# darrenjkt/SEE-VCN

Hardware: AMD Instinct MI355X
Metric: scenes/sec (VCN+voxel+spconv fwd+bwd) (higher is better)
Workload: dtype f32; 1 GPU; VCN_VC fwd on 64 objects x 1024 pts -> kNN surface select (k=30) -> largest DBSCAN cluster (eps 0.4) -> unique + replace (<0.1 m) into 16 KITTI-shaped 64-beam scenes (21.0k pts in range each) -> DynMeanVFE -> VoxelBackBone8x + HeightCompression fwd+bwd + SGD (BASELINE configs[1]+[2]); scenes_per_gpu=16, objects_per_gpu=64, points_per_object=1024, geometry=KITTI [0,-40,-3,70.4,40,1] @ [0.05,0.05,0.1] -> sparse [41,1600,1408], parallelism=dp1, input_side=side stream, one batch ahead (every step = 1 front + 1 compute)

## Files before the change

include/seevcn_hip.h:

```cpp
#ifndef SEEVCN_HIP_H
#define SEEVCN_HIP_H

#include <stddef.h>
#include <stdint.h>

#ifdef __cplusplus
extern "C" {
#endif

#define SV_OK 0
#define SV_ERR_ARG 1
#define SV_ERR_HIP 2

#define SV_ABI_VERSION 1

int sv_abi_version(void);
const char* sv_last_error(void);
int sv_measure_build(void);

size_t sv_index_persistent_bytes(int64_t ncells);
size_t sv_index_scratch_bytes(int64_t ncells);

size_t sv_voxelize_dynamic_scratch_bytes(int64_t num_points, int64_t ncells, int64_t capacity);
int sv_voxelize_dynamic(const float* points, int64_t num_points, int point_stride, int num_features,
// ... 293 lines not shown
int sv_weighted_smooth_l1_loss(const float* input, const float* target, const float* code_weights, const float* weights, int64_t n_rows,
                               int num_codes, float beta, const float* grad_out, float* out, void* stream);

int sv_center_assign_targets(const float* gt_boxes, int batch, int max_gt, int box_dim, int num_heads, int num_class,
                             const int32_t* cls_to_local, const int32_t* head_num_class, const int32_t* head_cls_offset, int total_cls,
                             int fm_w, int fm_h, float x_min, float y_min, float voxel_x, float voxel_y, float fm_stride,
                             int num_max_objs, float gaussian_overlap, int min_radius, float* heatmaps, float* target_boxes,
                             int64_t* inds, int64_t* masks, void* stream);

int sv_ball_query_batch(int batch, int n, int m, float radius, int nsample, const float* new_xyz, const float* xyz, int32_t* idx,
                        void* stream);
int sv_group_points_batch(int batch, int c, int n, int npoints, int nsample, const float* points, const int32_t* idx, float* out,
                          void* stream);
int sv_group_points_grad_batch(int batch, int c, int n, int npoints, int nsample, const float* grad_out, const int32_t* idx,
                               float* grad_points, void* stream);
int sv_gather_points_batch(int batch, int c, int n, int npoints, const float* points, const int32_t* idx, float* out, void* stream);
int sv_gather_points_grad_batch(int batch, int c, int n, int npoints, const float* grad_out, const int32_t* idx, float* grad_points,
                                void* stream);
int sv_three_nn_batch(int batch, int n, int m, const float* unknown, const float* known, float* dist2, int32_t* idx, void* stream);
int sv_three_interpolate_batch(int batch, int c, int m, int n, const float* points, const int32_t* idx, const float* weight, float* out,
                               void* stream);
int sv_three_interpolate_grad_batch(int batch, int c, int n, int m, const float* grad_out, const int32_t* idx, const float* weight,
                                    float* grad_points, void* stream);
size_t sv_group_points_grad_batch_ordered_scratch_bytes(int batch, int n, int npoints, int nsample);
int sv_group_points_grad_batch_ordered(int batch, int c, int n, int npoints, int nsample, const float* grad_out, const int32_t* idx,
                                       void* scratch, float* grad_points, void* stream);
size_t sv_gather_points_grad_batch_ordered_scratch_bytes(int batch, int n, int npoints);
int sv_gather_points_grad_batch_ordered(int batch, int c, int n, int npoints, const float* grad_out, const int32_t* idx, void* scratch,
                                        float* grad_points, void* stream);
size_t sv_three_interpolate_grad_batch_ordered_scratch_bytes(int batch, int n, int m);
int sv_three_interpolate_grad_batch_ordered(int batch, int c, int n, int m, const float* grad_out, const int32_t* idx, const float* weight,
                                            void* scratch, float* grad_points, void* stream);

#define SV_OP_WORDS 32
#define SV_OP_CONV_PLANNED 1
#define SV_OP_CONV_PLAIN 2
#define SV_OP_BN_FWD 3
#define SV_OP_BN_BWD 5
#define SV_OP_WGRAD 6
#define SV_OP_DGRAD_PLANNED_BN 7
#define SV_OP_WGRAD_DEFERRED 8
#define SV_OP_BN_FINALIZE 9
#define SV_OP_BN_APPLY 10
#define SV_OP_BN_STATS_LOCAL 11
#define SV_OP_BN_FINALIZE_GLOBAL 12
#define SV_OP_BN_BWD_SUMS_LOCAL 13
#define SV_OP_BN_BWD_APPLY_GLOBAL 14
#define SV_OP_BN_EVAL_COEF_BATCH 15
#define SV_OP_CONV_PLANNED_H16 16
#define SV_OP_NARROW_H16 17
int sv_run_ops(const int64_t* ops, int n_ops, void* stream);
int sv_run_ops_timed(const int64_t* ops, int n_ops, void* stream, float* ms);
int sv_run_ops_two_streams(const int64_t* ops, int n_ops, void* stream, void* side_stream);

size_t sv_batchnorm_scratch_bytes(int channels);
int sv_batchnorm_relu_forward(const float* x, int64_t n, int channels, const float* gamma, const float* beta, float* running_mean,
                              float* running_var, float momentum, float eps, int training, int relu, void* scratch, float* y,
                              float* save_mean, float* save_invstd, int64_t* num_batches_tracked, void* stream);
int sv_batchnorm_relu_forward_partial(const float* x, int64_t n, int channels, const float* gamma, const float* beta, float* running_mean,
                                      float* running_var, float momentum, float eps, int relu, void* scratch, int n_partials, float* y,
                                      float* save_mean, float* save_invstd, int64_t* num_batches_tracked, void* stream);
int sv_batchnorm_finalize_forward(const float* x , int64_t n, int channels, const float* gamma, const float* beta, float* running_mean, float* running_var,
                                  float momentum, float eps, void* scratch, int n_partials, float* coef, float* save_mean, float* save_invstd,
                                  int64_t* num_batches_tracked, void* stream);
int sv_batchnorm_eval_coef_batch(const int64_t* jobs_host, int n_jobs, void* stream);
int sv_batchnorm_apply(const float* x, int64_t n, int channels, const float* coef, int relu, float* y, void* stream);
int sv_batchnorm_relu_backward(const float* x, const float* dy, int64_t n, int channels, const float* gamma, const float* beta,
                               const float* save_mean, const float* save_invstd, int relu, void* scratch, float* dx, float* dgamma,
                               float* dbeta, void* stream);
int sv_batchnorm_relu_backward_partial(const float* x, const float* dy, int64_t n, int channels, const float* gamma, const float* beta,
                                       const float* save_mean, const float* save_invstd, int relu, void* scratch, int n_partials, float* dx,
                                       float* dgamma, float* dbeta, void* stream);
int sv_batchnorm_stats_local(const float* x, int64_t n, int channels, void* scratch, int n_partials, double* sums, void* stream);
int sv_batchnorm_finalize_global(const double* gathered, int world, int channels, const float* gamma, const float* beta, float* running_mean,
                                 float* running_var, float momentum, float eps, float* coef, float* save_mean, float* save_invstd,
                                 int64_t* num_batches_tracked, double* total_rows, void* stream);
int sv_batchnorm_backward_sums_local(const float* x, const float* dy, int64_t n, int channels, const float* gamma, const float* beta,
                                     const float* save_mean, const float* save_invstd, int relu, void* scratch, int n_partials, float* dgamma,
                                     float* dbeta, double* sums, void* stream);
int sv_batchnorm_backward_apply_global(const float* x, const float* dy, int64_t n, int channels, const float* gamma, const float* beta,
                                       const float* save_mean, const float* save_invstd, int relu, const double* gathered, int world,
                                       const double* total_rows, void* scratch, float* dx, void* stream);

int sv_gemm_bias_act_ragged(const float* A, int lda, const float* W, int ldw, const float* bias, const float* group_bias,
                            const int32_t* row_group, float* C, int ldc, float* group_max, int M, int N, int K, int act, float slope,
                            void* stream);
int sv_gemm_bias_act_ragged_dev(const float* A, int lda, const float* W, int ldw, const float* bias, const float* group_bias,
                                const int32_t* row_group, float* C, int ldc, float* group_max, int M_cap, const int32_t* m_dev, int N, int K,
                                int act, float slope, void* stream);
int sv_unique_rows(const float* x, int batch, int n, int32_t* uniq_idx, int32_t* counts, void* stream);
int sv_unique_rows_compact(const int32_t* uniq_idx, const int32_t* counts, int batch, int n, int64_t* sel, int32_t* row_group,
                           int32_t* total, void* stream);

int sv_chamfer_forward(const float* xyz1, const float* xyz2, int batch, int n, int m, float* dist1, float* dist2, int32_t* idx1,
                       int32_t* idx2, void* stream);
int sv_chamfer_backward(const float* xyz1, const float* xyz2, const int32_t* idx1, const int32_t* idx2, const float* grad_dist1,
                        const float* grad_dist2, int batch, int n, int m, float* grad_xyz1, float* grad_xyz2, void* stream);
size_t sv_chamfer_backward_ordered_scratch_bytes(int batch, int n, int m);
int sv_chamfer_backward_ordered(const float* xyz1, const float* xyz2, const int32_t* idx1, const int32_t* idx2, const float* grad_dist1,
                                const float* grad_dist2, int batch, int n, int m, void* scratch, float* grad_xyz1, float* grad_xyz2,
                                void* stream);

size_t sv_vcn_surface_select_scratch_bytes(int batch);
int sv_vcn_surface_select(const float* partial, const float* complete, int batch, int n_partial, int n_complete, int k,
                          int surface_pts, void* scratch, float* surface, int32_t* n_selected, void* stream);
int sv_vcn_largest_cluster(const float* points, int batch, int n, double eps, int min_points, int total_pts, float* out,
// ... 162 lines not shown
```

see-vcn_amd/_lib.py:

```python
import ctypes
import os

import torch

_HERE = os.path.dirname(os.path.abspath(__file__))
LIB_PATH = os.environ.get("SEEVCN_LIB") or os.path.join(_HERE, "lib", "libseevcn_hip.so")
HEADER_PATH = os.path.join(os.path.dirname(_HERE), "include", "seevcn_hip.h")

c_p = ctypes.c_void_p
c_i = ctypes.c_int
c_i64 = ctypes.c_int64
c_f = ctypes.c_float
c_d = ctypes.c_double
c_sz = ctypes.c_size_t

SIGNATURES = {
    "sv_abi_version": (c_i, []),
    "sv_last_error": (ctypes.c_char_p, []),
    "sv_measure_build": (c_i, []),
    "sv_index_persistent_bytes": (c_sz, [c_i64]),
    "sv_index_scratch_bytes": (c_sz, [c_i64]),
    "sv_voxelize_dynamic_scratch_bytes": (c_sz, [c_i64, c_i64, c_i64]),
    "sv_voxelize_dynamic": (c_i, [c_p, c_i64, c_i, c_i, c_p, c_p, c_p, c_i, c_p, c_p, c_p, c_p, c_p, c_i64, c_p, c_p]),
    "sv_mean_vfe": (c_i, [c_p, c_p, c_i64, c_i, c_i, c_p, c_p]),
# ... 153 lines not shown
    "sv_dedup_rows_scratch_bytes": (c_sz, [c_i64]),
    "sv_dedup_rows": (c_i, [c_p, c_i64, c_p, c_p]),
    "sv_points_near_set": (c_i, [c_p, c_i64, c_p, c_i64, c_i, c_d, c_p, c_p]),
    "sv_points_near_set_scratch_bytes": (c_sz, [c_i64]),
    "sv_points_near_set_boxed": (c_i, [c_p, c_i64, c_p, c_i64, c_i, c_d, c_p, c_p, c_p]),
    "sv_points_in_boxes_matrix": (c_i, [c_p, c_p, c_i, c_i, c_p, c_p]),
    "sv_crop_points_in_boxes": (c_i, [c_p, c_i64, c_i, c_p, c_i, c_i64, c_p, c_p, c_p]),
    "sv_project_lidar_to_image_kitti": (c_i, [c_p, c_i64, c_i, c_p, c_p, c_p, c_i, c_i, c_d, c_p, c_p, c_p, c_p]),
    "sv_project_lidar_to_image_camera": (c_i, [c_p, c_i64, c_i, c_p, c_p, c_p, c_i, c_i, c_i, c_p, c_p, c_p, c_p]),
    "sv_project_lidar_to_image_nuscenes": (c_i, [c_p, c_i64, c_i, c_p, c_p, c_p, c_i, c_i, c_d, c_p, c_p, c_p, c_p]),
    "sv_polygon_masks_scratch_bytes": (c_sz, [c_i, c_i, c_i]),
    "sv_polygons_to_masks": (c_i, [c_p, c_p, c_p, c_i, c_i, c_i, c_i, c_i, c_p, c_p, c_p]),
    "sv_polygons_to_masks_shrunk": (c_i, [c_p, c_p, c_p, c_p, c_i, c_i, c_i, c_i, c_i, c_p, c_p, c_p, c_p]),
    "sv_points_in_masks": (c_i, [c_p, c_p, c_i64, c_p, c_p, c_i, c_i, c_i, c_i64, c_p, c_p, c_p]),
    "sv_isolate_cluster_scratch_bytes": (c_i64, [c_i, c_i64]),
    "sv_isolate_largest_cluster": (c_i, [c_p, c_i, c_p, c_p, c_p, c_i, c_i64, c_d, c_d, c_d, c_d, c_d, c_i, c_i, c_p, c_p, c_p, c_p, c_p]),
    "sv_gemm_bias_act_ragged": (c_i, [c_p, c_i, c_p, c_i, c_p, c_p, c_p, c_p, c_i, c_p, c_i, c_i, c_i, c_i, c_f, c_p]),
    "sv_gemm_bias_act_ragged_dev": (c_i, [c_p, c_i, c_p, c_i, c_p, c_p, c_p, c_p, c_i, c_p, c_i, c_p, c_i, c_i, c_i, c_f, c_p]),
    "sv_unique_rows": (c_i, [c_p, c_i, c_i, c_p, c_p, c_p]),
    "sv_unique_rows_compact": (c_i, [c_p, c_p, c_i, c_i, c_p, c_p, c_p, c_p]),
    "sv_ball_query_batch": (c_i, [c_i, c_i, c_i, c_f, c_i, c_p, c_p, c_p, c_p]),
    "sv_group_points_batch": (c_i, [c_i, c_i, c_i, c_i, c_i, c_p, c_p, c_p, c_p]),
    "sv_group_points_grad_batch": (c_i, [c_i, c_i, c_i, c_i, c_i, c_p, c_p, c_p, c_p]),
    "sv_gather_points_batch": (c_i, [c_i, c_i, c_i, c_i, c_p, c_p, c_p, c_p]),
    "sv_gather_points_grad_batch": (c_i, [c_i, c_i, c_i, c_i, c_p, c_p, c_p, c_p]),
    "sv_three_nn_batch": (c_i, [c_i, c_i, c_i, c_p, c_p, c_p, c_p, c_p]),
    "sv_three_interpolate_batch": (c_i, [c_i, c_i, c_i, c_i, c_p, c_p, c_p, c_p, c_p]),
    "sv_three_interpolate_grad_batch": (c_i, [c_i, c_i, c_i, c_i, c_p, c_p, c_p, c_p, c_p]),
    "sv_group_points_grad_batch_ordered_scratch_bytes": (c_sz, [c_i, c_i, c_i, c_i]),
    "sv_group_points_grad_batch_ordered": (c_i, [c_i, c_i, c_i, c_i, c_i, c_p, c_p, c_p, c_p, c_p]),
    "sv_gather_points_grad_batch_ordered_scratch_bytes": (c_sz, [c_i, c_i, c_i]),
    "sv_gather_points_grad_batch_ordered": (c_i, [c_i, c_i, c_i, c_i, c_p, c_p, c_p, c_p, c_p]),
    "sv_three_interpolate_grad_batch_ordered_scratch_bytes": (c_sz, [c_i, c_i, c_i]),
    "sv_three_interpolate_grad_batch_ordered": (c_i, [c_i, c_i, c_i, c_i, c_p, c_p, c_p, c_p, c_p, c_p]),
    "sv_chamfer_forward":(c_i, [c_p, c_p, c_i, c_i, c_i, c_p, c_p, c_p, c_p, c_p]),
    "sv_chamfer_backward": (c_i, [c_p, c_p, c_p, c_p, c_p, c_p, c_i, c_i, c_i, c_p, c_p, c_p]),
    "sv_chamfer_backward_ordered_scratch_bytes": (c_sz, [c_i, c_i, c_i]),
    "sv_chamfer_backward_ordered": (c_i, [c_p, c_p, c_p, c_p, c_p, c_p, c_i, c_i, c_i, c_p, c_p, c_p, c_p]),
    "sv_batchnorm_scratch_bytes": (c_sz, [c_i]),
    "sv_batchnorm_relu_forward": (c_i, [c_p, c_i64, c_i, c_p, c_p, c_p, c_p, c_f, c_f, c_i, c_i, c_p, c_p, c_p, c_p, c_p, c_p]),
    "sv_batchnorm_relu_backward": (c_i, [c_p, c_p, c_i64, c_i, c_p, c_p, c_p, c_p, c_i, c_p, c_p, c_p, c_p, c_p]),
    "sv_batchnorm_relu_backward_partial": (c_i, [c_p, c_p, c_i64, c_i, c_p, c_p, c_p, c_p, c_i, c_p, c_i, c_p, c_p, c_p, c_p]),
    "sv_conv_next_input_norm": (c_i, [c_p, c_i]),
    "sv_batchnorm_finalize_forward": (c_i, [c_p, c_i64, c_i, c_p, c_p, c_p, c_p, c_f, c_f, c_p, c_i, c_p, c_p, c_p, c_p, c_p]),
    "sv_batchnorm_eval_coef_batch": (c_i, [c_p, c_i, c_p]),
    "sv_batchnorm_apply": (c_i, [c_p, c_i64, c_i, c_p, c_i, c_p, c_p]),
    "sv_batchnorm_stats_local": (c_i, [c_p, c_i64, c_i, c_p, c_i, c_p, c_p]),
    "sv_batchnorm_finalize_global": (c_i, [c_p, c_i, c_i, c_p, c_p, c_p, c_p, c_f, c_f, c_p, c_p, c_p, c_p, c_p, c_p]),
    "sv_batchnorm_backward_sums_local": (c_i, [c_p, c_p, c_i64, c_i, c_p, c_p, c_p, c_p, c_i, c_p, c_i, c_p, c_p, c_p, c_p]),
    "sv_batchnorm_backward_apply_global": (c_i, [c_p, c_p, c_i64, c_i, c_p, c_p, c_p, c_p, c_i, c_p, c_i, c_p, c_p, c_p, c_p]),
    "sv_run_ops": (c_i, [c_p, c_i, c_p]),
    "sv_run_ops_timed": (c_i, [c_p, c_i, c_p, c_p]),
    "sv_run_ops_two_streams": (c_i, [c_p, c_i, c_p, c_p]),
    "sv_anchor_decode": (c_i, [c_p, c_i64, c_p, c_p, c_i, c_i, c_f, c_f, c_p, c_p]),
    "sv_assign_targets_axis_aligned": (c_i, [c_p, c_i64, c_i, c_i, c_p, c_p, c_p, c_p, c_p, c_i, c_i, c_p, c_p, c_p, c_p, c_p]),
    "sv_anchor_decode_coded": (c_i, [c_p, c_i64, c_i, c_i, c_p, c_p, c_i, c_i, c_f, c_f, c_p, c_p]),
    "sv_assign_targets_axis_aligned_coded": (c_i, [c_p, c_i64, c_i, c_i, c_i, c_i, c_i, c_p, c_p, c_p, c_p, c_p, c_i, c_i, c_p, c_p, c_p, c_p, c_p]),
    "sv_focal_select_scratch_bytes": (c_sz, [c_i]),
    "sv_focal_select": (c_i, [c_p, c_p, c_i64, c_i, c_i, c_d, c_p, c_p, c_p]),
    "sv_focal_expand_scratch_bytes": (c_sz, [c_i64]),
    "sv_focal_expand": (c_i, [c_p, c_p, c_p, c_i64, c_i, c_p, c_d, c_p, c_p, c_p, c_p, c_i64, c_p, c_p]),
    "sv_focal_place": (c_i, [c_p, c_p, c_p, c_p, c_p, c_p, c_i64, c_i, c_i, c_i, c_d, c_i64, c_p, c_p, c_p, c_p]),
    "sv_focal_backward": (c_i, [c_p, c_p, c_p, c_p, c_p, c_p, c_p, c_p, c_p, c_i64, c_i, c_i, c_i, c_d, c_p, c_p, c_p, c_p]),
    "sv_kitti_eval_max_detections": (c_i, []),
    "sv_kitti_overlaps": (c_i, [c_p, c_p, c_p, c_p, c_p, c_i, c_i64, c_i, c_i, c_p, c_p]),
    "sv_kitti_match_scores": (c_i, [c_p, c_p, c_p, c_p, c_i, c_p, c_p, c_p, c_p, c_p, c_i, c_i64, c_i64, c_p, c_p, c_p]),
    "sv_kitti_thresholds": (c_i, [c_p, c_i64, c_p, c_p, c_i, c_p, c_p, c_p]),
    "sv_kitti_match_stats": (c_i, [c_p, c_p, c_p, c_p, c_i, c_p, c_p, c_p, c_p, c_p, c_i, c_i64, c_i64, c_p, c_p, c_i, c_i, c_p, c_p, c_p, c_p, c_p,
                                   c_p, c_p, c_p, c_p]),
    "sv_frustum_grid": (c_i, [c_p, c_p, c_p, c_i, c_i, c_i, c_i, c_p, c_i, c_d, c_d, c_i, c_p, c_p]),
    "sv_frustum_to_voxel": (c_i, [c_p, c_p, c_p, c_p, c_p, c_i, c_i, c_i, c_i, c_i, c_i, c_i, c_i, c_p, c_i, c_d, c_d, c_p, c_p]),
    "sv_frustum_to_voxel_grad_scratch_bytes": (c_sz, [c_i, c_i, c_i, c_i, c_i, c_i]),
    "sv_frustum_to_voxel_grad": (c_i, [c_p, c_p, c_p, c_p, c_p, c_p, c_i, c_i, c_i, c_i, c_i, c_i, c_i, c_i, c_p, c_i, c_d, c_d, c_p, c_p, c_p, c_p]),
    "sv_points_in_boxes_count": (c_i, [c_p, c_i, c_p, c_p, c_p, c_i, c_i, c_p, c_i, c_p, c_p, c_i, c_p, c_p]),
    "sv_object_scale_plan": (c_i, [c_p, c_i, c_p, c_p, c_p, c_i, c_p, c_i, c_p, c_p]),
    "sv_object_scale_points": (c_i, [c_p, c_i, c_p, c_p, c_p, c_i, c_i, c_p, c_i, c_p, c_p, c_p, c_p, c_p]),
    "sv_gt_sample_select": (c_i, [c_p, c_i, c_p, c_p, c_p, c_p, c_i, c_p, c_p, c_p, c_p, c_p, c_i, c_p, c_p]),
    "sv_gt_sample_paste": (c_i, [c_p, c_i, c_p, c_p, c_p, c_p, c_i, c_i, c_p, c_p, c_p, c_i, c_p, c_p, c_p, c_p, c_p, c_i, c_i, c_f, c_f, c_f, c_p]),
    "sv_world_transform_points": (c_i, [c_p, c_i, c_p, c_p, c_i, c_i, c_i64, c_i, c_p, c_p]),
    "sv_world_transform_boxes": (c_i, [c_p, c_i, c_p, c_p, c_p, c_i, c_i64, c_i, c_p, c_i, c_p]),
    "sv_augment_compact_scratch_bytes": (c_sz, [c_i, c_i]),
    "sv_augment_compact": (c_i, [c_p, c_i, c_p, c_p, c_p, c_i, c_i, c_p, c_p, c_i, c_p, c_p, c_p, c_p, c_i, c_p, c_p, c_p, c_p, c_p, c_i, c_p, c_p]),
    "sv_local_transform_plan": (c_i, [c_p, c_i, c_p, c_p, c_p, c_i, c_i, c_i64, c_i, c_p, c_p, c_p]),
    "sv_local_transform_points": (c_i, [c_p, c_i, c_p, c_p, c_p, c_i, c_i, c_p, c_p, c_i, c_i64, c_i, c_p, c_p]),
    "sv_world_frustum_dropout_scratch_bytes": (c_sz, [c_i, c_i]),
    "sv_world_frustum_dropout": (c_i, [c_p, c_i, c_p, c_p, c_p, c_i, c_i, c_p, c_i, c_p, c_p, c_p, c_i, c_i64, c_i, c_p, c_p, c_p]),
    "sv_get_pyramids": (c_i, [c_p, c_i, c_i, c_p, c_p]),
    "sv_pyramid_dropout": (c_i, [c_p, c_i, c_p, c_p, c_p, c_i, c_i, c_p, c_i, c_p, c_p, c_p, c_p, c_p]),
    "sv_pyramid_count": (c_i, [c_p, c_i, c_p, c_p, c_p, c_i, c_i, c_p, c_i, c_p, c_p, c_p, c_i, c_p, c_p, c_p, c_i, c_p]),
    "sv_pyramid_sparsify": (c_i, [c_p, c_i, c_p, c_p, c_p, c_p, c_i, c_p, c_i, c_i, c_p, c_i, c_p, c_i, c_p, c_p]),
    "sv_pyramid_swap": (c_i, [c_p, c_i, c_p, c_p, c_p, c_p, c_i, c_p, c_i, c_i, c_p, c_i, c_p, c_p]),
    "sv_bvh_scratch_bytes": (c_sz, [c_i64]),
    "sv_bvh_keys": (c_i, [c_p, c_i64, c_p, c_p, c_p, c_p]),
    "sv_bvh_build": (c_i, [c_p, c_p, c_p, c_i64, c_p, c_p, c_p, c_p, c_p]),
    "sv_cast_rays": (c_i, [c_p, c_p, c_i64, c_p, c_i64, c_p, c_p, c_p, c_p, c_p, c_p]),
    "sv_cast_pinhole": (c_i, [c_p, c_p, c_i64, c_p, c_i, c_i, c_i, c_p, c_p, c_p, c_p, c_p, c_p]),
    "sv_rays_pinhole": (c_i, [c_p, c_i, c_i, c_i, c_p, c_p]),
    "sv_ray_hit_points_scratch_bytes": (c_sz, [c_i, c_i, c_i]),
    "sv_ray_hit_points": (c_i, [c_p, c_p, c_i, c_i, c_i, c_p, c_p, c_p, c_p, c_p, c_p, c_p, c_p]),
    "sv_vc_rings": (c_i, [c_p, c_p, c_p, c_i, c_i, c_i, c_p, c_p, c_p, c_p, c_p]),
    "sv_vc_select": (c_i, [c_p, c_p, c_p, c_i, c_p, c_p, c_p, c_p, c_p]),
    "sv_vc_resample": (c_i, [c_p, c_p, c_p, c_i, c_p, c_i, c_p, c_p]),
    "sv_vc_pointwise": (c_i, [c_p, c_i64, c_p, c_i, c_p]),
    "sv_vc_object_scale": (c_i, [c_p, c_p, c_p, c_i, c_i, c_p, c_p]),
    "sv_vc_metrics_columns": (c_i, []),
    "sv_vc_metrics_tile": (c_i, []),
# ... 154 lines not shown
```

see-vcn_amd/csrc/common.h:

```cpp
#pragma once
#include <hip/hip_runtime.h>
#include <stdint.h>
#include <stdio.h>

#include "../../include/seevcn_hip.h"

#define SV_WAVE 64

void sv_set_error(const char* fmt, ...);

#define SV_CHECK_ARG(cond, ...)          \
  do {                                   \
    if (!(cond)) {                       \
      sv_set_error(__VA_ARGS__);         \
      return SV_ERR_ARG;                 \
    }                                    \
  } while (0)

#define SV_HIP(call)                                                               \
  do {                                                                             \
    hipError_t e_ = (call);                                                        \
    if (e_ != hipSuccess) {                                                        \
      sv_set_error("%s:%d: %s -> %s", __FILE__, __LINE__, #call, hipGetErrorString(e_)); \
      return SV_ERR_HIP;                                                           \
    }                                                                              \
  } while (0)

#define SV_LAUNCH_CHECK() SV_HIP(hipGetLastError())

static inline hipStream_t sv_stream(void* s) { return reinterpret_cast<hipStream_t>(s); }

static inline bool sv_on_device(const void* p) {
  hipPointerAttribute_t a;
  if (hipPointerGetAttributes(&a, p) != hipSuccess) {
    (void)hipGetLastError();
    return false;
  }
  return a.type == hipMemoryTypeDevice || a.type == hipMemoryTypeManaged;
}

static inline int sv_div_up(int64_t a, int64_t b) { return (int)((a + b - 1) / b); }

static inline int sv_grid_1d(int64_t n, int block, int max_blocks = 256 * 8) {
  int64_t g = (n + block - 1) / block;
  if (g < 1) g = 1;
  if (g > max_blocks) g = max_blocks;
  return (int)g;
}

#define SV_CHUNK_WORDS 32
#define SV_CHUNK_SHIFT 10

struct SvIndexView {
  uint2* words;
  int32_t* chunk_cnt;
  int32_t* chunk_base;
  int64_t ncells;
};

static inline int64_t sv_index_nwords(int64_t ncells) { return (ncells + 31) / 32; }
static inline int64_t sv_index_nchunks(int64_t ncells) { return (ncells + 1023) / 1024; }

static inline SvIndexView sv_index_view(void* ws, int64_t ncells) {
  SvIndexView v;
  int64_t nchunks = sv_index_nchunks(ncells);
  v.words = reinterpret_cast<uint2*>(ws);
  v.chunk_cnt = reinterpret_cast<int32_t*>(v.words + nchunks * SV_CHUNK_WORDS);
  v.chunk_base = v.chunk_cnt + nchunks;
  v.ncells = ncells;
  return v;
}

#ifdef __HIPCC__
__device__ __forceinline__ void sv_index_mark(const SvIndexView& ix, int64_t key) {
  const int64_t w = key >> 5;
  const uint32_t bit = 1u << (key & 31);
  const uint32_t old = atomicOr(&ix.words[w].x, bit);
  if (!(old & bit)) atomicAdd(&ix.chunk_cnt[key >> SV_CHUNK_SHIFT], 1);
}

__device__ __forceinline__ int32_t sv_index_rank_slow(const SvIndexView& ix, int64_t key, uint32_t* prefix_out) {
  const int64_t w = key >> 5;
  const int64_t w0 = (w / SV_CHUNK_WORDS) * SV_CHUNK_WORDS;
// ... 19 lines not shown
```

see-vcn_amd/csrc/norm.hip:

```cpp
#include <string.h>

#include "common.h"

#include "norm.h"

template <bool BWD>
__global__ __launch_bounds__(BN_THREADS) void k_bn_reduce(BnArgs a) {
  __shared__ float s_red[2][BN_THREADS * 4];
  const int tid = threadIdx.x, C4 = a.C >> 2;
  const int R = BN_THREADS / C4;
  const int c4 = tid % C4, rr = tid / C4;
  const bool active = rr < R;
  const int64_t rows_per_wg = (a.n + a.wgs - 1) / a.wgs;
  const int64_t r0 = (int64_t)blockIdx.x * rows_per_wg, r1 = min(a.n, r0 + rows_per_wg);
  float4 s0 = make_float4(0, 0, 0, 0), s1 = make_float4(0, 0, 0, 0);
  float4 mean = make_float4(0, 0, 0, 0), istd = mean, g = make_float4(1, 1, 1, 1), bt = mean;
  if (BWD && active) {
    mean = reinterpret_cast<const float4*>(a.save_mean)[c4], istd = reinterpret_cast<const float4*>(a.save_invstd)[c4];
    if (a.gamma) g = reinterpret_cast<const float4*>(a.gamma)[c4];
    if (a.beta) bt = reinterpret_cast<const float4*>(a.beta)[c4];
  }
  const float4 sc = make_float4(istd.x * g.x, istd.y * g.y, istd.z * g.z, istd.w * g.w);
  const float4 sh = make_float4(bn_shift(mean.x, sc.x, bt.x), bn_shift(mean.y, sc.y, bt.y), bn_shift(mean.z, sc.z, bt.z), bn_shift(mean.w, sc.w, bt.w));
  if (active) {
// ... 105 lines not shown
  for (int r = 1; r < world; ++r) t0 += gathered[r * stride + c], t1 += gathered[r * stride + a.C + c], n += gathered[r * stride + 2 * a.C];
  if (c == 0) {
    if (a.num_batches_tracked) *a.num_batches_tracked += 1;
    if (total_rows) *total_rows = n;
  }
  bn_finish_fwd(a, c, t0, t1, n);
}
__global__ void k_bn_coef_bwd_global(BnArgs a, const double* gathered, int world, const double* total_rows) {
  const int c = blockIdx.x * blockDim.x + threadIdx.x;
  if (c >= a.C) return;
  const size_t stride = 2 * (size_t)a.C;
  double t0 = gathered[c], t1 = gathered[a.C + c];
  for (int r = 1; r < world; ++r) t0 += gathered[r * stride + c], t1 += gathered[r * stride + a.C + c];
  bn_coef_bwd(a, c, t0, t1, *total_rows);
}

__global__ __launch_bounds__(BN_THREADS) void k_bn_apply_fwd(BnArgs a) {
  const int C4 = a.C >> 2;
  const int64_t total = a.n * C4;
  for (int64_t i = (int64_t)blockIdx.x * BN_THREADS + threadIdx.x; i < total; i += (int64_t)gridDim.x * BN_THREADS) {
    const int c4 = (int)(i % C4);
    const float4 v = reinterpret_cast<const float4*>(a.x)[i];
    const float4 sc = reinterpret_cast<const float4*>(a.coef)[c4], sh = reinterpret_cast<const float4*>(a.coef + a.C)[c4];
    float4 y = make_float4(bn_act(v.x, sc.x, sh.x), bn_act(v.y, sc.y, sh.y), bn_act(v.z, sc.z, sh.z), bn_act(v.w, sc.w, sh.w));
    if (a.relu) y.x = fmaxf(y.x, 0.f), y.y = fmaxf(y.y, 0.f), y.z = fmaxf(y.z, 0.f), y.w = fmaxf(y.w, 0.f);
    reinterpret_cast<float4*>(a.out)[i] = y;
  }
}

__global__ __launch_bounds__(BN_THREADS) void k_bn_apply_bwd(BnArgs a) {
  const int C4 = a.C >> 2;
  const int64_t total = a.n * C4;
  for (int64_t i = (int64_t)blockIdx.x * BN_THREADS + threadIdx.x; i < total; i += (int64_t)gridDim.x * BN_THREADS) {
    const int c4 = (int)(i % C4);
    const float4 v = reinterpret_cast<const float4*>(a.x)[i];
    float4 d = reinterpret_cast<const float4*>(a.dy)[i];
    const float4 k = reinterpret_cast<const float4*>(a.coef)[c4], md = reinterpret_cast<const float4*>(a.coef + a.C)[c4];
    const float4 mx = reinterpret_cast<const float4*>(a.coef + 2 * a.C)[c4], m = reinterpret_cast<const float4*>(a.coef + 3 * a.C)[c4];
    const float4 istd = reinterpret_cast<const float4*>(a.save_invstd)[c4];
    const float4 xh = make_float4((v.x - m.x) * istd.x, (v.y - m.y) * istd.y, (v.z - m.z) * istd.z, (v.w - m.w) * istd.w);
    if (a.relu) {
      const float4 g = a.gamma ? reinterpret_cast<const float4*>(a.gamma)[c4] : make_float4(1, 1, 1, 1);
      const float4 bt = a.beta ? reinterpret_cast<const float4*>(a.beta)[c4] : make_float4(0, 0, 0, 0);
      const float4 sc = make_float4(istd.x * g.x, istd.y * g.y, istd.z * g.z, istd.w * g.w);
      const float4 sh = make_float4(bn_shift(m.x, sc.x, bt.x), bn_shift(m.y, sc.y, bt.y), bn_shift(m.z, sc.z, bt.z), bn_shift(m.w, sc.w, bt.w));
      d.x = (bn_act(v.x, sc.x, sh.x) > 0.f) ? d.x : 0.f, d.y = (bn_act(v.y, sc.y, sh.y) > 0.f) ? d.y : 0.f;
      d.z = (bn_act(v.z, sc.z, sh.z) > 0.f) ? d.z : 0.f, d.w = (bn_act(v.w, sc.w, sh.w) > 0.f) ? d.w : 0.f;
    }
    reinterpret_cast<float4*>(a.out)[i] = make_float4(k.x * (d.x - md.x - xh.x * mx.x), k.y * (d.y - md.y - xh.y * mx.y),
                                                      k.z * (d.z - md.z - xh.z * mx.z), k.w * (d.w - md.w - xh.w * mx.w));
  }
}

static void bn_backward_tail(const BnArgs& a, hipStream_t st) {
  hipLaunchKernelGGL(k_bn_finalize<true>, dim3(a.C), dim3(BN_THREADS), 0, st, a);
  hipLaunchKernelGGL(k_bn_apply_bwd, dim3(sv_grid_1d(a.n * (a.C / 4), BN_THREADS)), dim3(BN_THREADS), 0, st, a);
}

__device__ __forceinline__ void bn_eval_coef(const float* gamma, const float* beta, const float* running_mean, const float* running_var, float eps,
                                             float* coef, int C, int c) {
  const float invstd = 1.f / sqrtf(running_var[c] + eps);
  const float gm = gamma ? gamma[c] : 1.f, bb = beta ? beta[c] : 0.f;
  coef[c] = invstd * gm;
  coef[C + c] = bb - running_mean[c] * invstd * gm;
}

__global__ void k_bn_eval_coef(BnArgs a) {
  const int c = blockIdx.x * blockDim.x + threadIdx.x;
  if (c >= a.C) return;
  bn_eval_coef(a.gamma, a.beta, a.running_mean, a.running_var, a.eps, a.coef, a.C, c);
}

struct BnEvalCoefJob {
  const float *gamma, *beta, *running_mean, *running_var;
  float* coef;
  int C;
  float eps;
};
constexpr int BN_EVAL_JOBS = 64;
struct BnEvalCoefBatch {
  BnEvalCoefJob j[BN_EVAL_JOBS];
};
static_assert(sizeof(BnEvalCoefBatch) <= 3900, "kernel argument block");

__global__ __launch_bounds__(128) void k_bn_eval_coef_batch(BnEvalCoefBatch b) {
  const BnEvalCoefJob& J = b.j[blockIdx.x];
  for (int c = threadIdx.x; c < J.C; c += 128) bn_eval_coef(J.gamma, J.beta, J.running_mean, J.running_var, J.eps, J.coef, J.C, c);
}

extern "C" int sv_batchnorm_eval_coef_batch(const int64_t* jobs_host, int n_jobs, void* stream) {
  SV_CHECK_ARG(n_jobs >= 0 && (jobs_host || n_jobs == 0), "sv_batchnorm_eval_coef_batch: bad arguments");
  if (n_jobs == 0) return SV_OK;
  for (int q = 0; q < n_jobs; ++q) {
    const int64_t* r = jobs_host + 8 * (size_t)q;
    SV_CHECK_ARG(r[2] && r[3] && r[4], "sv_batchnorm_eval_coef_batch: job %d: null pointer", q);
    SV_CHECK_ARG(r[5] >= 1 && r[5] <= BN_MAX_C, "sv_batchnorm_eval_coef_batch: job %d: 1..%d channels (got %lld)", q, BN_MAX_C, (long long)r[5]);
    SV_CHECK_ARG((uintptr_t)r[4] % 16 == 0, "sv_batchnorm_eval_coef_batch: job %d: coef_out must be 16-byte aligned", q);
  }
  hipStream_t st = sv_stream(stream);
  for (int q0 = 0; q0 < n_jobs; q0 += BN_EVAL_JOBS) {
    BnEvalCoefBatch b;
    const int nb = n_jobs - q0 < BN_EVAL_JOBS ? n_jobs - q0 : BN_EVAL_JOBS;
    for (int q = 0; q < nb; ++q) {
      const int64_t* r = jobs_host + 8 * (size_t)(q0 + q);
      BnEvalCoefJob& J = b.j[q];
      J.gamma = reinterpret_cast<const float*>((uintptr_t)r[0]), J.beta = reinterpret_cast<const float*>((uintptr_t)r[1]);
      J.running_mean = reinterpret_cast<const float*>((uintptr_t)r[2]), J.running_var = reinterpret_cast<const float*>((uintptr_t)r[3]);
      J.coef = reinterpret_cast<float*>((uintptr_t)r[4]);
      double eps;
// ... 155 lines not shown
}

extern "C" int sv_batchnorm_finalize_global(const double* gathered, int world, int channels, const float* gamma, const float* beta, float* running_mean,
                                            float* running_var, float momentum, float eps, float* coef, float* save_mean, float* save_invstd,
                                            int64_t* num_batches_tracked, double* total_rows, void* stream) {
  if (int rc = bn_common_check("sv_batchnorm_finalize_global", 1, channels)) return rc;
  SV_CHECK_ARG(world >= 1, "sv_batchnorm_finalize_global: world size %d", world);
  SV_CHECK_ARG(gathered && coef && save_mean && save_invstd && (uintptr_t)gathered % 8 == 0 && (uintptr_t)total_rows % 8 == 0,
               "sv_batchnorm_finalize_global: null or misaligned pointer");
  BnArgs a{};
  a.gamma = gamma, a.beta = beta, a.running_mean = running_mean, a.running_var = running_var;
  a.save_mean = save_mean, a.save_invstd = save_invstd, a.C = channels, a.momentum = momentum, a.eps = eps;
  a.num_batches_tracked = num_batches_tracked;
  a.coef = coef;
  hipLaunchKernelGGL(k_bn_finalize_global, dim3(sv_div_up(channels, 64)), dim3(64), 0, sv_stream(stream), a, gathered, world, total_rows);
  SV_LAUNCH_CHECK();
  return SV_OK;
}

extern "C" int sv_batchnorm_backward_sums_local(const float* x, const float* dy, int64_t n, int channels, const float* gamma, const float* beta,
                                                const float* save_mean, const float* save_invstd, int relu, void* scratch, int n_partials, float* dgamma,
                                                float* dbeta, double* sums, void* stream) {
  if (int rc = bn_common_check("sv_batchnorm_backward_sums_local", n, channels)) return rc;
  SV_CHECK_ARG(dgamma && dbeta && scratch && sums && (uintptr_t)sums % 8 == 0, "sv_batchnorm_backward_sums_local: null or misaligned pointer");
  SV_CHECK_ARG(n_partials >= 0 && n_partials <= BN_MAX_WGS, "sv_batchnorm_backward_sums_local: 0..%d partials (got %d)", BN_MAX_WGS, n_partials);
  SV_CHECK_ARG(n_partials > 0 || (x && dy && save_mean && save_invstd), "sv_batchnorm_backward_sums_local: the reduce pass needs x, dy, save_mean, save_invstd");
  BnArgs a{};
  a.x = x, a.dy = dy, a.gamma = gamma, a.beta = beta, a.dgamma = dgamma, a.dbeta = dbeta;
  a.save_mean = const_cast<float*>(save_mean), a.save_invstd = const_cast<float*>(save_invstd);
  a.n = n, a.C = channels, a.relu = relu;
  a.wgs = n_partials ? n_partials : bn_wgs(n, channels);
  bn_scratch(a, scratch);
  hipStream_t st = sv_stream(stream);
  if (!n_partials) hipLaunchKernelGGL(k_bn_reduce<true>, dim3(a.wgs), dim3(BN_THREADS), 0, st, a);
  hipLaunchKernelGGL(k_bn_sums_local<true>, dim3(channels), dim3(BN_THREADS), 0, st, a, sums);
  SV_LAUNCH_CHECK();
  return SV_OK;
}

extern "C" int sv_batchnorm_backward_apply_global(const float* x, const float* dy, int64_t n, int channels, const float* gamma, const float* beta,
                                                  const float* save_mean, const float* save_invstd, int relu, const double* gathered, int world,
                                                  const double* total_rows, void* scratch, float* dx, void* stream) {
  if (int rc = bn_common_check("sv_batchnorm_backward_apply_global", n, channels)) return rc;
  SV_CHECK_ARG(world >= 1, "sv_batchnorm_backward_apply_global: world size %d", world);
  SV_CHECK_ARG(x && dy && dx && save_mean && save_invstd && scratch && gathered && total_rows && (uintptr_t)gathered % 8 == 0 && (uintptr_t)total_rows % 8 == 0,
               "sv_batchnorm_backward_apply_global: null or misaligned pointer");
  BnArgs a{};
  a.x = x, a.dy = dy, a.out = dx, a.gamma = gamma, a.beta = beta;
  a.save_mean = const_cast<float*>(save_mean), a.save_invstd = const_cast<float*>(save_invstd);
  a.n = n, a.C = channels, a.relu = relu;
  bn_scratch(a, scratch);
  hipStream_t st = sv_stream(stream);
  hipLaunchKernelGGL(k_bn_coef_bwd_global, dim3(sv_div_up(channels, 64)), dim3(64), 0, st, a, gathered, world, total_rows);
  hipLaunchKernelGGL(k_bn_apply_bwd, dim3(sv_grid_1d(n * (channels / 4), BN_THREADS)), dim3(BN_THREADS), 0, st, a);
  SV_LAUNCH_CHECK();
  return SV_OK;
}

void sv_bn_finalize_fwd(const BnArgs& a, hipStream_t st) { hipLaunchKernelGGL(k_bn_finalize<false>, dim3(a.C), dim3(BN_THREADS), 0, st, a); }
void sv_bn_finalize_bwd(const BnArgs& a, hipStream_t st) { hipLaunchKernelGGL(k_bn_finalize<true>, dim3(a.C), dim3(BN_THREADS), 0, st, a); }
```

see-vcn_amd/csrc/sequencer.hip:

```cpp
#include <string.h>

#include "common.h"

namespace {
inline double as_double(int64_t bits) {
  double d;
  memcpy(&d, &bits, sizeof d);
  return d;
}
template <typename T>
inline T* ptr_of(int64_t v) { return reinterpret_cast<T*>(static_cast<uintptr_t>(v)); }
}

struct SeqEvents {
  hipEvent_t fork = nullptr, join = nullptr;
  int create() {
    SV_HIP(hipEventCreateWithFlags(&fork, hipEventDisableTiming));
    SV_HIP(hipEventCreateWithFlags(&join, hipEventDisableTiming));
    return SV_OK;
  }
  ~SeqEvents() {
    if (fork) (void)hipEventDestroy(fork);
    if (join) (void)hipEventDestroy(join);
  }
};

static int run_ops(const int64_t* ops, int n_ops, void* stream, void* side_stream, float* ms = nullptr);

extern "C" int sv_run_ops(const int64_t* ops, int n_ops, void* stream) { return run_ops(ops, n_ops, stream, nullptr); }

extern "C" int sv_run_ops_timed(const int64_t* ops, int n_ops, void* stream, float* ms) {
  SV_CHECK_ARG(ms || n_ops == 0, "sv_run_ops_timed: null output");
  return run_ops(ops, n_ops, stream, nullptr, ms);
}

extern "C" int sv_run_ops_two_streams(const int64_t* ops, int n_ops, void* stream, void* side_stream) {
  SV_CHECK_ARG(side_stream && side_stream != stream, "sv_run_ops_two_streams: needs a second stream");
  return run_ops(ops, n_ops, stream, side_stream);
}

static int run_ops(const int64_t* ops, int n_ops, void* stream, void* side_stream, float* ms) {
  SV_CHECK_ARG(n_ops >= 0 && (ops || n_ops == 0), "sv_run_ops: null list");
  struct Stamps {
    hipEvent_t* ev = nullptr;
    int n = 0;
    ~Stamps() {
      for (int q = 0; q < n; ++q) (void)hipEventDestroy(ev[q]);
      delete[] ev;
    }
  } stamps;
  if (ms) {
    stamps.ev = new hipEvent_t[n_ops + 1];
    for (; stamps.n <= n_ops; ++stamps.n) SV_HIP(hipEventCreate(&stamps.ev[stamps.n]));
    SV_HIP(hipEventRecord(stamps.ev[0], sv_stream(stream)));
  }
  hipStream_t st_main = sv_stream(stream), st_side = side_stream ? sv_stream(side_stream) : nullptr;
  bool side_used = false;
  SeqEvents ev;
  if (st_side) {
    if (int rc = ev.create()) return rc;
  }
  auto fork_side = [&]() -> int {
    SV_HIP(hipEventRecord(ev.fork, st_main));
    side_used = true;
    SV_HIP(hipStreamWaitEvent(st_side, ev.fork, 0));
    return SV_OK;
  };
  void* const wstream = side_stream ? side_stream : stream;
  constexpr int MAX_DEFERRED = 64;
  int64_t deferred[MAX_DEFERRED * 10];
  int n_deferred = 0, fail = SV_OK;
  for (int k = 0; k < n_ops; ++k) {
    const int64_t* o = ops + (size_t)k * SV_OP_WORDS;
    const int64_t* i = o + 1;
    const int64_t* n = o + 9;
    const int64_t* f = o + 13;
    const int64_t* p = o + 17;
    int rc = SV_OK;
    switch ((int)o[0]) {
      case SV_OP_CONV_PLANNED:
        if (p[12]) sv_conv_next_input_norm(ptr_of<const float>(p[12]), (int)i[6]);
        rc = sv_sparse_conv_gather_gemm_planned(ptr_of<const float>(p[0]), n[0], ptr_of<const int32_t>(p[1]), ptr_of<const int32_t>(p[2]),
                                                ptr_of<const int32_t>(p[3]), ptr_of<const int32_t>(p[4]), (int)i[0], ptr_of<const float>(p[5]),
                                                ptr_of<float>(p[6]), n[1], (int)i[1], (int)i[2], (int)i[3], ptr_of<const float>(p[7]),
                                                ptr_of<const float>(p[8]), ptr_of<const float>(p[9]), ptr_of<const float>(p[10]), (int)i[4], (int)i[5],
                                                ptr_of<float>(p[11]), stream);
        break;
      case SV_OP_CONV_PLAIN:
        rc = sv_sparse_conv_gather_gemm(ptr_of<const float>(p[0]), n[0], ptr_of<const int32_t>(p[1]), ptr_of<const float>(p[2]), ptr_of<float>(p[3]), n[1],
                                        (int)i[0], (int)i[1], (int)i[2], ptr_of<const float>(p[4]), ptr_of<const float>(p[5]), ptr_of<const float>(p[6]),
                                        ptr_of<const float>(p[7]), (int)i[3], stream);
        break;
      case SV_OP_BN_FWD:
        if (i[3] > 0)
          rc = sv_batchnorm_relu_forward_partial(ptr_of<const float>(p[0]), n[0], (int)i[0], ptr_of<const float>(p[1]), ptr_of<const float>(p[2]),
                                                 ptr_of<float>(p[3]), ptr_of<float>(p[4]), (float)as_double(f[0]), (float)as_double(f[1]), (int)i[2],
                                                 ptr_of<void>(p[5]), (int)i[3], ptr_of<float>(p[6]), ptr_of<float>(p[7]), ptr_of<float>(p[8]),
                                                 ptr_of<int64_t>(p[9]), stream);
        else
          rc = sv_batchnorm_relu_forward(ptr_of<const float>(p[0]), n[0], (int)i[0], ptr_of<const float>(p[1]), ptr_of<const float>(p[2]), ptr_of<float>(p[3]),
                                         ptr_of<float>(p[4]), (float)as_double(f[0]), (float)as_double(f[1]), (int)i[1], (int)i[2], ptr_of<void>(p[5]),
                                         ptr_of<float>(p[6]), ptr_of<float>(p[7]), ptr_of<float>(p[8]), ptr_of<int64_t>(p[9]), stream);
        break;
      case SV_OP_DGRAD_PLANNED_BN:
        rc = sv_sparse_conv_dgrad_planned_bn(ptr_of<const float>(p[0]), n[0], ptr_of<const int32_t>(p[1]), ptr_of<const int32_t>(p[2]),
                                             ptr_of<const int32_t>(p[3]), ptr_of<const int32_t>(p[4]), (int)i[0], ptr_of<const float>(p[5]),
                                             ptr_of<float>(p[6]), n[1], (int)i[1], (int)i[2], (int)i[3], (int)i[4], ptr_of<const float>(p[7]),
                                             ptr_of<const float>(p[8]), ptr_of<const float>(p[9]), ptr_of<const float>(p[10]), ptr_of<const float>(p[11]),
                                             (int)i[5], ptr_of<float>(p[12]), stream);
        break;
      case SV_OP_BN_BWD:
        if (i[2] > 0)
          rc = sv_batchnorm_relu_backward_partial(ptr_of<const float>(p[0]), ptr_of<const float>(p[1]), n[0], (int)i[0], ptr_of<const float>(p[2]),
                                                  ptr_of<const float>(p[3]), ptr_of<const float>(p[4]), ptr_of<const float>(p[5]), (int)i[1],
                                                  ptr_of<void>(p[6]), (int)i[2], ptr_of<float>(p[7]), ptr_of<float>(p[8]), ptr_of<float>(p[9]), stream);
        else
        rc = sv_batchnorm_relu_backward(ptr_of<const float>(p[0]), ptr_of<const float>(p[1]), n[0], (int)i[0], ptr_of<const float>(p[2]),
                                        ptr_of<const float>(p[3]), ptr_of<const float>(p[4]), ptr_of<const float>(p[5]), (int)i[1], ptr_of<void>(p[6]),
                                        ptr_of<float>(p[7]), ptr_of<float>(p[8]), ptr_of<float>(p[9]), stream);
        break;
      case SV_OP_BN_FINALIZE: {
#if SEEVCN_MEASURE
        static const int skip_after = getenv("SEEVCN_DEBUG_SKIP_FINALIZE") ? atoi(getenv("SEEVCN_DEBUG_SKIP_FINALIZE")) : 0;
        static int calls = 0;
        if (skip_after > 0 && ++calls > skip_after && !p[9]) break;
#endif
        rc = sv_batchnorm_finalize_forward(ptr_of<const float>(p[9]), n[0], (int)i[0], ptr_of<const float>(p[0]), ptr_of<const float>(p[1]), ptr_of<float>(p[2]), ptr_of<float>(p[3]),
                                           (float)as_double(f[0]), (float)as_double(f[1]), ptr_of<void>(p[4]), (int)i[1], ptr_of<float>(p[5]), ptr_of<float>(p[6]),
                                           ptr_of<float>(p[7]), ptr_of<int64_t>(p[8]), stream);
        break;
      }
      case SV_OP_BN_APPLY:
        rc = sv_batchnorm_apply(ptr_of<const float>(p[0]), n[0], (int)i[0], ptr_of<const float>(p[1]), (int)i[1], ptr_of<float>(p[2]), stream);
        break;
      case SV_OP_BN_STATS_LOCAL:
        rc = sv_batchnorm_stats_local(ptr_of<const float>(p[0]), n[0], (int)i[0], ptr_of<void>(p[1]), (int)i[1], ptr_of<double>(p[2]), stream);
        break;
      case SV_OP_BN_FINALIZE_GLOBAL:
        rc = sv_batchnorm_finalize_global(ptr_of<const double>(p[0]), (int)i[1], (int)i[0], ptr_of<const float>(p[1]), ptr_of<const float>(p[2]), ptr_of<float>(p[3]),
                                          ptr_of<float>(p[4]), (float)as_double(f[0]), (float)as_double(f[1]), ptr_of<float>(p[5]), ptr_of<float>(p[6]),
                                          ptr_of<float>(p[7]), ptr_of<int64_t>(p[8]), ptr_of<double>(p[9]), stream);
        break;
      case SV_OP_BN_BWD_SUMS_LOCAL:
        rc = sv_batchnorm_backward_sums_local(ptr_of<const float>(p[0]), ptr_of<const float>(p[1]), n[0], (int)i[0], ptr_of<const float>(p[2]),
                                              ptr_of<const float>(p[3]), ptr_of<const float>(p[4]), ptr_of<const float>(p[5]), (int)i[1], ptr_of<void>(p[6]),
                                              (int)i[2], ptr_of<float>(p[7]), ptr_of<float>(p[8]), ptr_of<double>(p[9]), stream);
        break;
      case SV_OP_BN_BWD_APPLY_GLOBAL:
        rc = sv_batchnorm_backward_apply_global(ptr_of<const float>(p[0]), ptr_of<const float>(p[1]), n[0], (int)i[0], ptr_of<const float>(p[2]),
                                                ptr_of<const float>(p[3]), ptr_of<const float>(p[4]), ptr_of<const float>(p[5]), (int)i[1],
                                                ptr_of<const double>(p[7]), (int)i[2], ptr_of<const double>(p[8]), ptr_of<void>(p[6]), ptr_of<float>(p[9]), stream);
        break;
      case SV_OP_BN_EVAL_COEF_BATCH:
        rc = sv_batchnorm_eval_coef_batch(ptr_of<const int64_t>(p[0]), (int)i[0], stream);
        break;
      case SV_OP_CONV_PLANNED_H16:
        rc = sv_sparse_conv_gather_gemm_planned_h16(ptr_of<const void>(p[0]), n[0], ptr_of<const int32_t>(p[1]), ptr_of<const int32_t>(p[2]),
                                                    ptr_of<const int32_t>(p[3]), ptr_of<const void>(p[4]), ptr_of<void>(p[5]), (int)i[4], n[1], (int)i[0],
                                                    (int)i[1], (int)i[2], ptr_of<const float>(p[6]), ptr_of<const float>(p[7]), ptr_of<const float>(p[8]),
                                                    ptr_of<const void>(p[9]), (int)i[3], stream);
        break;
      case SV_OP_NARROW_H16:
        rc = sv_narrow_h16(ptr_of<const float>(p[0]), n[0], ptr_of<void>(p[1]), stream);
        break;
      case SV_OP_WGRAD:
        if (st_side && (rc = fork_side()) != SV_OK) break;
        if (p[6]) sv_conv_next_input_norm(ptr_of<const float>(p[6]), (int)i[4]);
        if (p[5])
          rc = sv_sparse_conv_wgrad_planned(ptr_of<const float>(p[0]), i[3], ptr_of<const int32_t>(p[1]), ptr_of<const float>(p[2]), ptr_of<float>(p[3]), n[0],
                                            (int)i[0], (int)i[1], (int)i[2], n[1], n[2], n[3], ptr_of<const void>(p[5]), ptr_of<void>(p[4]), wstream);
        else
        rc = sv_sparse_conv_wgrad_strided(ptr_of<const float>(p[0]), i[3], ptr_of<const int32_t>(p[1]), ptr_of<const float>(p[2]), ptr_of<float>(p[3]), n[0],
                                          (int)i[0], (int)i[1], (int)i[2], n[1], n[2], n[3], ptr_of<void>(p[4]), wstream);
        break;
      case SV_OP_WGRAD_DEFERRED:
        if (st_side && (rc = fork_side()) != SV_OK) break;
        if (n_deferred == MAX_DEFERRED) {
          rc = sv_sparse_conv_wgrad_reduce_batch(deferred, n_deferred, wstream);
          n_deferred = 0;
          if (rc != SV_OK) break;
        }
        if (p[6]) sv_conv_next_input_norm(ptr_of<const float>(p[6]), (int)i[4]);
        if (p[5])
          rc = sv_sparse_conv_wgrad_planned_stage1(ptr_of<const float>(p[0]), i[3], ptr_of<const int32_t>(p[1]), ptr_of<const float>(p[2]), ptr_of<float>(p[3]), n[0],
                                                   (int)i[0], (int)i[1], (int)i[2], n[1], n[2], n[3], ptr_of<const void>(p[5]), ptr_of<void>(p[4]),
                                                   deferred + 10 * n_deferred, wstream);
        else
        rc = sv_sparse_conv_wgrad_stage1(ptr_of<const float>(p[0]), i[3], ptr_of<const int32_t>(p[1]), ptr_of<const float>(p[2]), ptr_of<float>(p[3]), n[0],
                                         (int)i[0], (int)i[1], (int)i[2], n[1], n[2], n[3], ptr_of<void>(p[4]), deferred + 10 * n_deferred, wstream);
        ++n_deferred;
        break;
      default:
        sv_set_error("sv_run_ops: unknown operation %lld at position %d", (long long)o[0], k);
        rc = SV_ERR_ARG;
        break;
    }
    if (rc != SV_OK) {
      fail = rc;
      break;
    }
    if (ms) SV_HIP(hipEventRecord(stamps.ev[k + 1], st_main));
  }
  int rc = fail;
  sv_conv_next_input_norm(nullptr, 0);
  if (rc == SV_OK && n_deferred > 0) rc = sv_sparse_conv_wgrad_reduce_batch(deferred, n_deferred, wstream);
  if (ms && rc == SV_OK) {
    SV_HIP(hipStreamSynchronize(st_main));
    for (int k = 0; k < n_ops; ++k) SV_HIP(hipEventElapsedTime(&ms[k], stamps.ev[k], stamps.ev[k + 1]));
  }
  if (side_used) {
    hipError_t e = hipEventRecord(ev.join, st_side);
    if (e == hipSuccess) e = hipStreamWaitEvent(st_main, ev.join, 0);
    if (e != hipSuccess) {
      (void)hipStreamSynchronize(st_side);
      if (rc == SV_OK) {
        sv_set_error("sv_run_ops_two_streams: joining the side stream failed: %s", hipGetErrorString(e));
        rc = SV_ERR_HIP;
      }
    }
  }
  return rc;
}
```

Before: 4526 scenes/sec.

## Fork side-stream wgrad from kernel-completion event bound via hipExtLaunchKernel

The BN-backward apply kernel that precedes a weight-gradient op is launched with hipExtLaunchKernel carrying a completion event. The side stream waits on that event directly instead of on a separately recorded fork event, which trims the host work and the stream dependency at each wgrad fork. Each fork now gets its own event. The batched reduction of deferred wgrad partials is issued before the last deferred wgrad forks, so it can overlap sooner. This adds per-call event creation and thread-local launch state that must stay consistent with the launch path.

```diff
diff --git a/include/seevcn_hip.h b/include/seevcn_hip.h
--- a/include/seevcn_hip.h
+++ b/include/seevcn_hip.h
@@ -369,6 +369,7 @@
 int sv_run_ops(const int64_t* ops, int n_ops, void* stream);
 int sv_run_ops_timed(const int64_t* ops, int n_ops, void* stream, float* ms);
 int sv_run_ops_two_streams(const int64_t* ops, int n_ops, void* stream, void* side_stream);
+int sv_next_launch_event_pending(void);
 
 size_t sv_batchnorm_scratch_bytes(int channels);
 int sv_batchnorm_relu_forward(const float* x, int64_t n, int channels, const float* gamma, const float* beta, float* running_mean,
diff --git a/see-vcn_amd/_lib.py b/see-vcn_amd/_lib.py
--- a/see-vcn_amd/_lib.py
+++ b/see-vcn_amd/_lib.py
@@ -229,6 +229,7 @@
     "sv_run_ops": (c_i, [c_p, c_i, c_p]),
     "sv_run_ops_timed": (c_i, [c_p, c_i, c_p, c_p]),
     "sv_run_ops_two_streams": (c_i, [c_p, c_i, c_p, c_p]),
+    "sv_next_launch_event_pending": (c_i, []),
     "sv_anchor_decode": (c_i, [c_p, c_i64, c_p, c_p, c_i, c_i, c_f, c_f, c_p, c_p]),
     "sv_assign_targets_axis_aligned": (c_i, [c_p, c_i64, c_i, c_i, c_p, c_p, c_p, c_p, c_p, c_i, c_i, c_p, c_p, c_p, c_p, c_p]),
     "sv_anchor_decode_coded": (c_i, [c_p, c_i64, c_i, c_i, c_p, c_p, c_i, c_i, c_f, c_f, c_p, c_p]),
diff --git a/see-vcn_amd/csrc/common.h b/see-vcn_amd/csrc/common.h
--- a/see-vcn_amd/csrc/common.h
+++ b/see-vcn_amd/csrc/common.h
@@ -29,6 +29,11 @@
 #define SV_LAUNCH_CHECK() SV_HIP(hipGetLastError())
 
 static inline hipStream_t sv_stream(void* s) { return reinterpret_cast<hipStream_t>(s); }
+
+void sv_next_launch_event(hipEvent_t ev);
+hipEvent_t sv_take_launch_event();
+void sv_launch_event_bound();
+bool sv_launch_event_was_bound();
 
 static inline bool sv_on_device(const void* p) {
   hipPointerAttribute_t a;
diff --git a/see-vcn_amd/csrc/norm.hip b/see-vcn_amd/csrc/norm.hip
--- a/see-vcn_amd/csrc/norm.hip
+++ b/see-vcn_amd/csrc/norm.hip
@@ -181,9 +181,23 @@
   }
 }
 
+static void launch_bn_apply_bwd(const BnArgs& a, hipStream_t st) {
+  const dim3 grid(sv_grid_1d(a.n * (a.C / 4), BN_THREADS)), block(BN_THREADS);
+  if (hipEvent_t ev = sv_take_launch_event()) {
+    BnArgs arg = a;
+    void* args[] = {&arg};
+    if (hipExtLaunchKernel(reinterpret_cast<const void*>(k_bn_apply_bwd), grid, block, args, 0, st, nullptr, ev, 0) == hipSuccess) {
+      sv_launch_event_bound();
+      return;
+    }
+    (void)hipGetLastError();
+  }
+  hipLaunchKernelGGL(k_bn_apply_bwd, grid, block, 0, st, a);
+}
+
 static void bn_backward_tail(const BnArgs& a, hipStream_t st) {
   hipLaunchKernelGGL(k_bn_finalize<true>, dim3(a.C), dim3(BN_THREADS), 0, st, a);
-  hipLaunchKernelGGL(k_bn_apply_bwd, dim3(sv_grid_1d(a.n * (a.C / 4), BN_THREADS)), dim3(BN_THREADS), 0, st, a);
+  launch_bn_apply_bwd(a, st);
 }
 
 __device__ __forceinline__ void bn_eval_coef(const float* gamma, const float* beta, const float* running_mean, const float* running_var, float eps,
@@ -445,7 +459,7 @@
   bn_scratch(a, scratch);
   hipStream_t st = sv_stream(stream);
   hipLaunchKernelGGL(k_bn_coef_bwd_global, dim3(sv_div_up(channels, 64)), dim3(64), 0, st, a, gathered, world, total_rows);
-  hipLaunchKernelGGL(k_bn_apply_bwd, dim3(sv_grid_1d(n * (channels / 4), BN_THREADS)), dim3(BN_THREADS), 0, st, a);
+  launch_bn_apply_bwd(a, st);
   SV_LAUNCH_CHECK();
   return SV_OK;
 }
diff --git a/see-vcn_amd/csrc/sequencer.hip b/see-vcn_amd/csrc/sequencer.hip
--- a/see-vcn_amd/csrc/sequencer.hip
+++ b/see-vcn_amd/csrc/sequencer.hip
@@ -1,4 +1,6 @@
 #include <string.h>
+
+#include <vector>
 
 #include "common.h"
 
@@ -12,15 +14,42 @@
 inline T* ptr_of(int64_t v) { return reinterpret_cast<T*>(static_cast<uintptr_t>(v)); }
 }
 
+namespace {
+struct NextLaunchEvent {
+  hipEvent_t ev = nullptr;
+  bool bound = false;
+};
+thread_local NextLaunchEvent g_next_event;
+}
+void sv_next_launch_event(hipEvent_t ev) { g_next_event.ev = ev, g_next_event.bound = false; }
+hipEvent_t sv_take_launch_event() {
+  const hipEvent_t ev = g_next_event.ev;
+  g_next_event.ev = nullptr;
+  return ev;
+}
+void sv_launch_event_bound() { g_next_event.bound = true; }
+bool sv_launch_event_was_bound() {
+  const bool b = g_next_event.bound;
+  g_next_event = NextLaunchEvent{};
+  return b;
+}
+extern "C" int sv_next_launch_event_pending(void) { return g_next_event.ev != nullptr; }
+
 struct SeqEvents {
-  hipEvent_t fork = nullptr, join = nullptr;
+  std::vector<hipEvent_t> forks;
+  hipEvent_t join = nullptr;
   int create() {
-    SV_HIP(hipEventCreateWithFlags(&fork, hipEventDisableTiming));
     SV_HIP(hipEventCreateWithFlags(&join, hipEventDisableTiming));
     return SV_OK;
   }
+  int next_fork(hipEvent_t* ev) {
+    SV_HIP(hipEventCreateWithFlags(ev, hipEventDisableTiming));
+    forks.push_back(*ev);
+    return SV_OK;
+  }
   ~SeqEvents() {
-    if (fork) (void)hipEventDestroy(fork);
+    sv_next_launch_event(nullptr);
+    for (hipEvent_t e : forks) (void)hipEventDestroy(e);
     if (join) (void)hipEventDestroy(join);
   }
 };
@@ -61,15 +90,48 @@
     if (int rc = ev.create()) return rc;
   }
   auto fork_side = [&]() -> int {
-    SV_HIP(hipEventRecord(ev.fork, st_main));
+    hipEvent_t fork;
+    if (int rc = ev.next_fork(&fork)) return rc;
+    SV_HIP(hipEventRecord(fork, st_main));
     side_used = true;
-    SV_HIP(hipStreamWaitEvent(st_side, ev.fork, 0));
-    return SV_OK;
-  };
+    SV_HIP(hipStreamWaitEvent(st_side, fork, 0));
+    return SV_OK;
+  };
+  auto code_at = [&](int k) -> int { return k >= 0 && k < n_ops ? (int)ops[(size_t)k * SV_OP_WORDS] : 0; };
+  auto is_wgrad = [&](int k) -> bool { return code_at(k) == SV_OP_WGRAD || code_at(k) == SV_OP_WGRAD_DEFERRED; };
+  hipEvent_t bound_fork = nullptr;
+  int forked = -1;
   void* const wstream = side_stream ? side_stream : stream;
   constexpr int MAX_DEFERRED = 64;
   int64_t deferred[MAX_DEFERRED * 10];
   int n_deferred = 0, fail = SV_OK;
+  int last_deferred = -1;
+  if (st_side && !ms)
+    for (int k = 0; k < n_ops; ++k)
+      if (code_at(k) == SV_OP_WGRAD_DEFERRED) last_deferred = k;
+  auto early_sums = [&](int k) -> int {
+    if (k != last_deferred || n_deferred == 0) return SV_OK;
+    const int rc = sv_sparse_conv_wgrad_reduce_batch(deferred, n_deferred, wstream);
+    n_deferred = 0;
+    return rc;
+  };
+  auto offer_fork = [&](int k) -> int {
+    bound_fork = nullptr;
+    if (!st_side || ms || !is_wgrad(k + 1)) return SV_OK;
+    if (int rc = early_sums(k + 1)) return rc;
+    if (int rc = ev.next_fork(&bound_fork)) return rc;
+    sv_next_launch_event(bound_fork);
+    return SV_OK;
+  };
+  auto settle_fork = [&](int k, int op_rc) -> int {
+    if (!bound_fork) return SV_OK;
+    const bool bound = sv_launch_event_was_bound();
+    if (op_rc != SV_OK || !bound) return SV_OK;
+    side_used = true;
+    SV_HIP(hipStreamWaitEvent(st_side, bound_fork, 0));
+    forked = k + 1;
+    return SV_OK;
+  };
   for (int k = 0; k < n_ops; ++k) {
     const int64_t* o = ops + (size_t)k * SV_OP_WORDS;
     const int64_t* i = o + 1;
@@ -110,6 +172,7 @@
                                              (int)i[5], ptr_of<float>(p[12]), stream);
         break;
       case SV_OP_BN_BWD:
+        if ((rc = offer_fork(k)) != SV_OK) break;
         if (i[2] > 0)
           rc = sv_batchnorm_relu_backward_partial(ptr_of<const float>(p[0]), ptr_of<const float>(p[1]), n[0], (int)i[0], ptr_of<const float>(p[2]),
                                                   ptr_of<const float>(p[3]), ptr_of<const float>(p[4]), ptr_of<const float>(p[5]), (int)i[1],
@@ -118,6 +181,7 @@
         rc = sv_batchnorm_relu_backward(ptr_of<const float>(p[0]), ptr_of<const float>(p[1]), n[0], (int)i[0], ptr_of<const float>(p[2]),
                                         ptr_of<const float>(p[3]), ptr_of<const float>(p[4]), ptr_of<const float>(p[5]), (int)i[1], ptr_of<void>(p[6]),
                                         ptr_of<float>(p[7]), ptr_of<float>(p[8]), ptr_of<float>(p[9]), stream);
+        if (int frc = settle_fork(k, rc)) rc = rc != SV_OK ? rc : frc;
         break;
       case SV_OP_BN_FINALIZE: {
 #if SEEVCN_MEASURE
@@ -147,9 +211,11 @@
                                               (int)i[2], ptr_of<float>(p[7]), ptr_of<float>(p[8]), ptr_of<double>(p[9]), stream);
         break;
       case SV_OP_BN_BWD_APPLY_GLOBAL:
+        if ((rc = offer_fork(k)) != SV_OK) break;
         rc = sv_batchnorm_backward_apply_global(ptr_of<const float>(p[0]), ptr_of<const float>(p[1]), n[0], (int)i[0], ptr_of<const float>(p[2]),
                                                 ptr_of<const float>(p[3]), ptr_of<const float>(p[4]), ptr_of<const float>(p[5]), (int)i[1],
                                                 ptr_of<const double>(p[7]), (int)i[2], ptr_of<const double>(p[8]), ptr_of<void>(p[6]), ptr_of<float>(p[9]), stream);
+        if (int frc = settle_fork(k, rc)) rc = rc != SV_OK ? rc : frc;
         break;
       case SV_OP_BN_EVAL_COEF_BATCH:
         rc = sv_batchnorm_eval_coef_batch(ptr_of<const int64_t>(p[0]), (int)i[0], stream);
@@ -164,7 +230,7 @@
         rc = sv_narrow_h16(ptr_of<const float>(p[0]), n[0], ptr_of<void>(p[1]), stream);
         break;
       case SV_OP_WGRAD:
-        if (st_side && (rc = fork_side()) != SV_OK) break;
+        if (st_side && forked != k && (rc = fork_side()) != SV_OK) break;
         if (p[6]) sv_conv_next_input_norm(ptr_of<const float>(p[6]), (int)i[4]);
         if (p[5])
           rc = sv_sparse_conv_wgrad_planned(ptr_of<const float>(p[0]), i[3], ptr_of<const int32_t>(p[1]), ptr_of<const float>(p[2]), ptr_of<float>(p[3]), n[0],
@@ -174,7 +240,8 @@
                                           (int)i[0], (int)i[1], (int)i[2], n[1], n[2], n[3], ptr_of<void>(p[4]), wstream);
         break;
       case SV_OP_WGRAD_DEFERRED:
-        if (st_side && (rc = fork_side()) != SV_OK) break;
+        if ((rc = early_sums(k)) != SV_OK) break;
+        if (st_side && forked != k && (rc = fork_side()) != SV_OK) break;
         if (n_deferred == MAX_DEFERRED) {
           rc = sv_sparse_conv_wgrad_reduce_batch(deferred, n_deferred, wstream);
           n_deferred = 0;
@@ -203,6 +270,7 @@
   }
   int rc = fail;
   sv_conv_next_input_norm(nullptr, 0);
+  sv_next_launch_event(nullptr);
   if (rc == SV_OK && n_deferred > 0) rc = sv_sparse_conv_wgrad_reduce_batch(deferred, n_deferred, wstream);
   if (ms && rc == SV_OK) {
     SV_HIP(hipStreamSynchronize(st_main));
```

Result: no change. 4534 scenes/sec, median of 2 (+0.2%).
